# pairlab/SlotFormer

Measured on AMD Instinct MI355X. Metric: rollout frames/sec at B=32, 128x128, 7 slots, 6+50 steps (SAVi-encode + SlotFormer rollout), higher is better.
Workload: dtype f32 storage; matmul/conv on split-bf16 MFMA (bf16x3: hi*hi+hi*lo+lo*hi, f32 accumulate)

## Files before the change

### slotformer_amd/csrc/layer_tok.hip

```cpp
#include "../../include/slotformer_hip.h"
#include "sf_internal.h"
#include "layer_fused.h"
#include "layer_tok_common.h"
#include <stdlib.h>

namespace {
constexpr int LT_NT = 256, LT_D = 256, LT_F = 1024, LT_NH = 8, LT_TOK = 128, LT_MAXL = 8;
constexpr int LT_STAGE = 32 * 1024, LT_RING = 3;
constexpr int LT_NST_ATT = 4 * LT_NH, LT_NST = LT_NST_ATT + 2 * (LT_F / 32);
constexpr int LT_KV = LT_RING * LT_STAGE;
constexpr int LT_VT = LT_KV + 16 * 1024;
constexpr int LT_PAR = LT_KV + 32 * 1024;
constexpr int P_LN1G = 0, P_LN1B = 256, P_BQKV = 512, P_BO = 1280, P_LN2G = 1536, P_LN2B = 1792, P_B1 = 2048, P_B2 = 3072, P_N = 3328;
constexpr size_t LT_LDS = (size_t)LT_PAR + (size_t)P_N * 4;
constexpr size_t LT_BLOB = (size_t)LT_NST * LT_STAGE + (size_t)P_N * 4;
static_assert(LT_LDS <= 160 * 1024, "LDS budget");

struct LtArgs {
  const float* x;
  const float* ring;
  const float* pe;
  float* y;
  const char* blob[LT_MAXL];
  float eps;
  int nl, B, L, vpw, RF, N, f0, dbg_ts;
};
}

__device__ long long lt_ts[16];
#define LTS(i) do { if (A.dbg_ts && blockIdx.x == 0 && threadIdx.x == 0) lt_ts[i] = wall_clock64(); } while (0)

template <int MODE>
__global__ __launch_bounds__(LT_NT) void layer_tok_kernel(LtArgs A) {
  extern __shared__ __attribute__((aligned(16))) char smem[];
  float* P = (float*)(smem + LT_PAR);
  const int t = threadIdx.x, lane = t & 63;
  const int wave = __builtin_amdgcn_readfirstlane(t >> 6);
  const int n = lane & 31, h = lane >> 5;
  const int L = A.L;
  const int v0 = blockIdx.x * A.vpw;
  const int nvalid = min(A.vpw, A.B - v0) * L;
  const int tl = wave * 32 + n;
  const int te = min(tl, nvalid - 1);
  const int vl = te / L, tok = te - vl * L;
  const long long row = (long long)(v0 + vl) * L + tok;
  LTS(0);
  f32x16 X[8];
  if constexpr (MODE == 0) {
    const float* xr = A.x + row * LT_D + 4 * h;
#pragma unroll
    for (int ob = 0; ob < 8; ++ob)
#pragma unroll
      for (int g = 0; g < 4; ++g) {
        const f32x4 v = *(const f32x4*)(xr + 32 * ob + 8 * g);
#pragma unroll
        for (int q = 0; q < 4; ++q) X[ob][4 * g + q] = v[q];
      }
  } else {
    const int fr = tok / A.N, sl = tok - fr * A.N;
    const float* rr = A.ring + (((long long)(v0 + vl) * A.RF + (A.f0 + fr) % A.RF) * A.N + sl) * LT_D + 4 * h;
    const float* pr = A.pe + (long long)tok * LT_D + 4 * h;
#pragma unroll
    for (int ob = 0; ob < 8; ++ob)
#pragma unroll
      for (int g = 0; g < 4; ++g) {
        const f32x4 v = *(const f32x4*)(rr + 32 * ob + 8 * g);
#pragma unroll
        for (int q = 0; q < 4; ++q) X[ob][4 * g + q] = v[q];
      }
    __builtin_amdgcn_sched_barrier(0);
#pragma unroll
    for (int ob = 0; ob < 8; ++ob) {
#pragma unroll
      for (int g = 0; g < 4; ++g) {
        const f32x4 v = *(const f32x4*)(pr + 32 * ob + 8 * g);
#pragma unroll
        for (int q = 0; q < 4; ++q) X[ob][4 * g + q] += v[q];
      }
      __builtin_amdgcn_sched_barrier(0);
    }
  }
  const unsigned wlane = (unsigned)(wave * 8 * 1024 + lane * 16);
  char* const wdst = smem + (wave * 8) * 1024;
  int cur = 0;
  int cs = -2;
  const char* base_cur = A.blob[0];
  const char* base_nxt = A.blob[0];
  bool last_layer = false;
  auto stage_src = [&]() -> const char* {
    const int t2 = cs + 2;
    const bool wrap = t2 >= LT_NST;
    const char* b = wrap ? base_nxt : base_cur;
    const int so = wrap ? (last_layer ? LT_NST - 1 : t2 - LT_NST) : t2;
    ++cs;
    return b + (size_t)so * LT_STAGE + wlane;
  };
  {
    const char* s0 = stage_src();
    const char* s1 = stage_src();
    LtRing R0{nullptr, s0, wdst}, R1{nullptr, s1, wdst + LT_STAGE};
#pragma unroll
    for (int f = 0; f < 8; ++f) lt_dma(R0, f);
#pragma unroll
    for (int f = 0; f < 8; ++f) lt_dma(R1, f);
  }
#ifdef LT_STAMPS
  long long c_wait = 0, c_bar = 0, c_last = 0, c_work = 0;
#endif
  auto stage_begin = [&]() -> LtRing {
#ifdef LT_STAMPS
    const long long c0 = __builtin_readcyclecounter();
    if (c_last) c_work += c0 - c_last;
#endif
#ifdef LT_NODMA
    asm volatile("s_waitcnt vmcnt(0)" ::: "memory");
#else
    asm volatile("s_waitcnt vmcnt(8)" ::: "memory");
#endif
    asm volatile("s_waitcnt lgkmcnt(0)" ::: "memory");
#ifdef LT_STAMPS
    const long long c1 = __builtin_readcyclecounter();
#endif
#ifndef LT_NOBAR
    __builtin_amdgcn_s_barrier();
#endif
    asm volatile("" ::: "memory");
#ifdef LT_STAMPS
    c_last = __builtin_readcyclecounter();
    c_wait += c1 - c0;
    c_bar += c_last - c1;
#endif
    const int nb = cur == 0 ? 2 : cur - 1;
    LtRing R{smem + cur * LT_STAGE + lane * 16, stage_src(), wdst + nb * LT_STAGE};
#ifdef LT_BURST
#pragma unroll
    for (int f = 0; f < 8; ++f) lt_dma_now(R, f);
#endif
    cur = cur == 2 ? 0 : cur + 1;
    return R;
  };
  const int wf = min(wave * 32, nvalid - 1);
  const int kb0 = ((wf / L) * L) >> 5;
  const int d0 = 32 * kb0 + 4 * h - vl * L;
  const char* pb;
  {
    unsigned pbo = (unsigned)(LT_PAR + 16 * h);
    asm volatile("" : "+v"(pbo));
    pb = smem + pbo;
  }
  char* const kwr = smem + LT_KV + wave * 1024 + lane * 16;
  char* const vwr = smem + LT_VT + wave * 4096 + lane * 16;
  const char* krd[3];
  const char* vrd[3];
#pragma unroll
  for (int kbi = 0; kbi < 3; ++kbi) {
    const int kb = min(kb0 + kbi, 3);
    krd[kbi] = smem + LT_KV + kb * 1024 + lane * 16;
    vrd[kbi] = smem + LT_VT + kb * 4096 + lane * 16;
  }
  const float qscale = 0.2550348616841918f;
  constexpr float NEG = -3.0e38f;
  LTS(1);

#pragma unroll 1
  for (int l = 0; l < A.nl; ++l) {
    cs = 0;
    base_cur = A.blob[l];
    last_layer = l + 1 >= A.nl;
    base_nxt = A.blob[last_layer ? l : l + 1];
    __syncthreads();
    {
      const float* vsrc = (const float*)(A.blob[l] + (size_t)LT_NST * LT_STAGE);
      for (int i = t; i < P_N / 4; i += LT_NT) *(f32x4*)(P + 4 * i) = *(const f32x4*)(vsrc + 4 * i);
    }
    __syncthreads();
    if (l == 0) LTS(2);
    bf16x8 xh[16], xl[16];
    lt_layernorm<P_LN1G, P_LN1B>(X, pb, h, A.eps, xh, xl);
    lt_add_vec<P_BO>(X, pb);
    if (l == 0) LTS(3);
    f32x16 qa, ka, va, S[3], O;
    bf16x8 qh[2], ql[2], ph[3][2], pl[3][2], oh[2], ol[2];
    float mx0 = NEG, mx1 = NEG, mx = 0.f, sm = 0.f, rinv = 0.f;
    auto zero16 = [](f32x16& a) {
#pragma unroll
      for (int r = 0; r < 16; ++r) a[r] = 0.f;
    };
    int hq = 0;
    auto mask_chunk = [&](int c) {
      const int kbi = c >> 1;
#pragma unroll
      for (int rr = 0; rr < 8; ++rr) {
        const int r = 8 * (c & 1) + rr;
        const bool ok = (unsigned)(d0 + 32 * kbi + 8 * (r >> 2) + (r & 3)) < (unsigned)L;
        const float v = ok ? S[kbi][r] : NEG;
        S[kbi][r] = v;
        if (rr & 1) mx1 = fmaxf(mx1, v); else mx0 = fmaxf(mx0, v);
      }
    };
    auto exp_chunk = [&](int c) {
      const int kbi = c >> 1;
      float s0 = 0.f, s1 = 0.f;
#pragma unroll
      for (int rr = 0; rr < 8; ++rr) {
        const int r = 8 * (c & 1) + rr;
#ifdef LT_EXPF
        const float e = __expf((S[kbi][r] - mx) * 0.6931471805599453f);
#else
        const float e = __builtin_amdgcn_exp2f(S[kbi][r] - mx);
#endif
        S[kbi][r] = e;
        if (rr & 1) s1 += e; else s0 += e;
      }
      sm += s0 + s1;
    };
    auto psplit_chunk = [&](int c) { split8(quad(S[c >> 1], 2 * (c & 1)), quad(S[c >> 1], 2 * (c & 1) + 1), ph[c >> 1][c & 1], pl[c >> 1][c & 1]); };
    auto kconv = [&](int s) {
      const float* bk = (const float*)pb + P_BQKV + 256 + 32 * hq;
      bf16x8 fh, fl;
      split8(quad(ka, 2 * s) + *(const f32x4*)(bk + 16 * s), quad(ka, 2 * s + 1) + *(const f32x4*)(bk + 16 * s + 8), fh, fl);
      *(bf16x8*)(kwr + (s * 2) * 4096) = fh;
      *(bf16x8*)(kwr + (s * 2 + 1) * 4096) = fl;
    };
    auto qconv = [&](int s) {
      const float* bq = (const float*)pb + P_BQKV + 32 * hq;
      split8((quad(qa, 2 * s) + *(const f32x4*)(bq + 16 * s)) * qscale, (quad(qa, 2 * s + 1) + *(const f32x4*)(bq + 16 * s + 8)) * qscale, qh[s], ql[s]);
    };
    auto vconv = [&](int s) {
      const float bv = P[P_BQKV + 512 + 32 * hq + n];
      bf16x8 fh, fl;
      split8(quad(va, 2 * s) + bv, quad(va, 2 * s + 1) + bv, fh, fl);
      *(bf16x8*)(vwr + (s * 2) * 1024) = fh;
      *(bf16x8*)(vwr + (s * 2 + 1) * 1024) = fl;
    };
    auto oconv = [&](int s) { split8(quad(O, 2 * s) * rinv, quad(O, 2 * s + 1) * rinv, oh[s], ol[s]); };
    auto scores = [&]() {
      bf16x8 kh[3][2], kl[3][2];
#pragma unroll
      for (int kbi = 0; kbi < 3; ++kbi)
#pragma unroll
        for (int s = 0; s < 2; ++s) {
          kh[kbi][s] = *(const bf16x8*)(krd[kbi] + (s * 2) * 4096);
          kl[kbi][s] = *(const bf16x8*)(krd[kbi] + (s * 2 + 1) * 4096);
        }
#pragma unroll
      for (int kbi = 0; kbi < 3; ++kbi) zero16(S[kbi]);
#pragma unroll
      for (int s = 0; s < 2; ++s) {
#pragma unroll
        for (int kbi = 0; kbi < 3; ++kbi) { S[kbi] = LT_MFMA(kh[kbi][s], ql[s], S[kbi]); LT_PIN(); }
#pragma unroll
        for (int kbi = 0; kbi < 3; ++kbi) { S[kbi] = LT_MFMA(kl[kbi][s], qh[s], S[kbi]); LT_PIN(); }
#pragma unroll
        for (int kbi = 0; kbi < 3; ++kbi) { S[kbi] = LT_MFMA(kh[kbi][s], qh[s], S[kbi]); LT_PIN(); }
      }
      mx0 = mx1 = NEG;
      sm = 0.f;
    };
    auto pv = [&]() {
      f32x16 Op[3];
      bf16x8 vh[3][2], vlo[3][2];
#pragma unroll
      for (int kbi = 0; kbi < 3; ++kbi)
#pragma unroll
        for (int s = 0; s < 2; ++s) {
          vh[kbi][s] = *(const bf16x8*)(vrd[kbi] + (s * 2) * 1024);
          vlo[kbi][s] = *(const bf16x8*)(vrd[kbi] + (s * 2 + 1) * 1024);
        }
#pragma unroll
      for (int kbi = 0; kbi < 3; ++kbi) zero16(Op[kbi]);
#pragma unroll
      for (int s = 0; s < 2; ++s) {
#pragma unroll
        for (int kbi = 0; kbi < 3; ++kbi) { Op[kbi] = LT_MFMA(vh[kbi][s], pl[kbi][s], Op[kbi]); LT_PIN(); }
#pragma unroll
        for (int kbi = 0; kbi < 3; ++kbi) { Op[kbi] = LT_MFMA(vlo[kbi][s], ph[kbi][s], Op[kbi]); LT_PIN(); }
#pragma unroll
        for (int kbi = 0; kbi < 3; ++kbi) { Op[kbi] = LT_MFMA(vh[kbi][s], ph[kbi][s], Op[kbi]); LT_PIN(); }
      }
#pragma unroll
      for (int r = 0; r < 16; ++r) O[r] = (Op[0][r] + Op[1][r]) + Op[2][r];
    };
    auto sideD = [&](int g) {
      if (g < 6) mask_chunk(g);
      if (g == 6) mx = lt_xmax(fmaxf(mx0, mx1), h);
      if (g == 7) exp_chunk(0);
    };
    auto sideA = [&](int g) {
      if (g == 0) { exp_chunk(1); exp_chunk(2); }
      if (g == 1) { exp_chunk(3); exp_chunk(4); }
      if (g == 2) { exp_chunk(5); rinv = 1.0f / lt_xsum(sm, h); psplit_chunk(0); }
      if (g == 3) { psplit_chunk(1); psplit_chunk(2); }
      if (g == 4) { psplit_chunk(3); psplit_chunk(4); }
      if (g == 5) psplit_chunk(5);
    };
    {
      const LtRing R = stage_begin();
      lt_row_product<false, 0>(R, xh, xl, qa, LtNoSide{});
    }
    {
      const LtRing R = stage_begin();
      lt_row_product<false, 0>(R, xh, xl, ka, LtNoSide{});
    }
    {
      const LtRing R = stage_begin();
      lt_row_product<true, 5>(R, xh, xl, va, [&](int g) {
        if (g < 2) kconv(g);
        else if (g < 4) qconv(g - 2);
      });
      vconv(0);
      vconv(1);
    }
#pragma unroll 1
    for (hq = 1; hq < LT_NH; ++hq) {
      {
        const LtRing R = stage_begin();
        scores();
          lt_row_product<false, 6>(R, xh, xl, qa, sideD);
      }
      {
        const LtRing R = stage_begin();
          lt_row_product<false, 6>(R, xh, xl, ka, sideA);
        pv();
      }
      {
        const LtRing R = stage_begin();
          lt_row_product<true, 5>(R, xh, xl, va, [&](int g) {
          if (g < 2) kconv(g);
          else if (g < 4) qconv(g - 2);
          else if (g < 6) oconv(g - 4);
        });
      }
      {
        const LtRing R = stage_begin();
        lt_kslice_product<5>(R, oh, ol, X, [&](int g) {
          if (g < 2) vconv(g);
        });
      }
    }
    asm volatile("s_waitcnt lgkmcnt(0)" ::: "memory");
    __builtin_amdgcn_s_barrier();
    asm volatile("" ::: "memory");
    scores();
#pragma unroll
    for (int g = 0; g < 8; ++g) sideD(g);
#pragma unroll
    for (int g = 0; g < 6; ++g) sideA(g);
    pv();
    oconv(0);
    oconv(1);
    {
      const LtRing R = stage_begin();
      lt_kslice_product<0>(R, oh, ol, X, LtNoSide{});
    }
    if (l == 0) LTS(4);
#ifdef LT_STAMPS
    if (l == 0 && blockIdx.x == 0 && threadIdx.x == 0) { lt_ts[8] = c_wait; lt_ts[9] = c_bar; lt_ts[10] = c_work; }
#endif
    lt_layernorm<P_LN2G, P_LN2B>(X, pb, h, A.eps, xh, xl);
    lt_add_vec<P_B2>(X, pb);
    if (l == 0) LTS(5);
    f32x16 Ha, Hb;
    bf16x8 hh[2], hl[2];
    f32x4 b1q[4];
    auto b1_load = [&](int blk) {
      const float* b1 = (const float*)pb + P_B1 + 32 * blk;
#pragma unroll
      for (int g = 0; g < 4; ++g) b1q[g] = *(const f32x4*)(b1 + 8 * g);
    };
    auto hconv = [&](const f32x16& Hx, int s) {
      const f32x4 z4 = {0.f, 0.f, 0.f, 0.f};
      const f32x4 u0 = __builtin_elementwise_max(quad(Hx, 2 * s) + b1q[2 * s], z4);
      const f32x4 u1 = __builtin_elementwise_max(quad(Hx, 2 * s + 1) + b1q[2 * s + 1], z4);
      split8(u0, u1, hh[s], hl[s]);
    };
    auto ffn_step = [&](f32x16& Hn, const f32x16& Hp, int j) {
      {
        const LtRing R = stage_begin();
        lt_row_product<false, 4>(R, xh, xl, Hn, [&](int g) {
          if (g >= 1 && g < 3) hconv(Hp, g - 1);
        });
        asm volatile("" : "+v"(hh[0]), "+v"(hh[1]), "+v"(hl[0]), "+v"(hl[1]));
      }
      {
        const LtRing R = stage_begin();
        b1_load(j);
        lt_kslice_product<0>(R, hh, hl, X, LtNoSide{});
      }
    };
    {
      const LtRing R = stage_begin();
      b1_load(0);
      lt_row_product<false, 0>(R, xh, xl, Ha, LtNoSide{});
    }
    ffn_step(Hb, Ha, 1);
#pragma unroll 1
    for (int j = 2; j < LT_F / 32; j += 2) {
      ffn_step(Ha, Hb, j);
      ffn_step(Hb, Ha, j + 1);
    }
    hconv(Hb, 0);
    hconv(Hb, 1);
    {
      const LtRing R = stage_begin();
      lt_kslice_product<0>(R, hh, hl, X, LtNoSide{});
    }
    if (l == 0) LTS(6);
#ifdef LT_STAMPS
    if (l == 0 && blockIdx.x == 0 && threadIdx.x == 0) { lt_ts[11] = c_wait; lt_ts[12] = c_bar; lt_ts[13] = c_work; }
#endif
  }
  asm volatile("s_waitcnt vmcnt(0)" ::: "memory");
  if (tl < nvalid) {
    float* yr = A.y + row * LT_D + 4 * h;
#pragma unroll
    for (int ob = 0; ob < 8; ++ob)
#pragma unroll
      for (int g = 0; g < 4; ++g) *(f32x4*)(yr + 32 * ob + 8 * g) = quad(X[ob], g);
  }
  LTS(7);
}

extern "C" int sf_debug_read_ts_layer_tok(long long* out16) {
  hipError_t e = hipMemcpyFromSymbol(out16, HIP_SYMBOL(lt_ts), sizeof(long long) * 16);
  return e == hipSuccess ? 0 : (int)e;
}

extern "C" size_t sf_layer_tok_packed_bytes(void) { return LT_BLOB; }
extern "C" size_t sf_layer_tok_packed_bytes_ex(int d_model, int num_heads, int ffn) {
  if (d_model == LT_D && num_heads == LT_NH && ffn == LT_F) return LT_BLOB;
  return sf_layer_tok128_shape(d_model, num_heads, ffn) ? sf_layer_tok128_packed_bytes() : 0;
}

extern "C" int sf_pack_layer_tok_weights(const sf_tfm_layer* w, void* packed, int d_model, int num_heads, int ffn, void* stream) {
  SF_REQUIRE(w && packed, "sf_pack_layer_tok_weights: null pointer");
  SF_REQUIRE(w->in_proj_w && w->out_proj_w && w->lin1_w && w->lin2_w && w->norm1_g && w->norm1_b && w->in_proj_b && w->out_proj_b && w->norm2_g &&
                 w->norm2_b && w->lin1_b && w->lin2_b, "sf_pack_layer_tok_weights: null weight");
  hipStream_t st = (hipStream_t)stream;
  if (sf_layer_tok128_shape(d_model, num_heads, ffn)) return sf_pack_layer_tok128(w, packed, st);
  SF_REQUIRE(d_model == LT_D && num_heads == LT_NH && ffn == LT_F, "sf_pack_layer_tok_weights: (d_model, heads, ffn) = (256, 8, 1024) or (128, 8, 512) only");
  const int total = LT_NST * 32 * 64;
  hipLaunchKernelGGL((pack_layer_tok_kernel<LT_D, LT_F>), dim3((total + 255) / 256), dim3(256), 0, st, w->in_proj_w, w->out_proj_w, w->lin1_w, w->lin2_w, (uint4*)packed);
  SF_CHECK_LAUNCH();
  float* vec = (float*)((char*)packed + (size_t)LT_NST * LT_STAGE);
  const struct {
    const float* src;
    int off, n;
  } parts[8] = {{w->norm1_g, P_LN1G, 256}, {w->norm1_b, P_LN1B, 256}, {w->in_proj_b, P_BQKV, 768}, {w->out_proj_b, P_BO, 256},
                {w->norm2_g, P_LN2G, 256}, {w->norm2_b, P_LN2B, 256}, {w->lin1_b, P_B1, 1024},   {w->lin2_b, P_B2, 256}};
  for (const auto& p : parts) {
    const hipError_t e = hipMemcpyAsync(vec + p.off, p.src, (size_t)p.n * 4, hipMemcpyDeviceToDevice, st);
    if (e != hipSuccess) return sf_set_err((int)e, hipGetErrorString(e), __FILE__, __LINE__);
  }
  return 0;
}

int sf_layer_tok_vpw(int L) {
  if (L < 1 || L > 96) return 0;
  for (int vpw = LT_TOK / L; vpw >= 1; --vpw) {
    const int nvalid = vpw * L;
    bool ok = true;
    for (int w = 0; w < 4 && ok; ++w) {
      const int wf = w * 32 < nvalid ? w * 32 : nvalid - 1, wl = w * 32 + 31 < nvalid ? w * 32 + 31 : nvalid - 1;
      const int kb0 = ((wf / L) * L) >> 5, kb1 = (((wl / L) * L) + L - 1) >> 5;
      ok = kb1 - kb0 + 1 <= 3;
    }
    if (ok) return vpw;
  }
  return 0;
}
bool sf_layer_tok_ok(int L) { return sf_layer_tok_vpw(L) > 0; }

int sf_layer_tok_ex(int mode, const float* xin, const float* ring, int ring_frames, int nslots, int f0, const float* pe, const sf_tfm_layer* layers, int nl,
                    float eps, float* y, int B, int L, hipStream_t st) {
  bool ok = layers && nl >= 1 && nl <= LT_MAXL && sf_layer_tok_ok(L) && B >= 1 && y && (mode == 0 ? xin != nullptr : (ring && pe && nslots >= 1 && ring_frames >= 1));
  for (int l = 0; ok && l < nl; ++l) ok = layers[l].tok_packed != nullptr;
  if (!ok)
    return sf_set_err(-1, "invalid argument: the token-stationary layers need sf_pack_layer_tok_weights fragments, 1..8 layers and 1 <= L <= 96 rows per video", __FILE__, __LINE__);
  static const int dbg = sf_dbg("lt");
  LtArgs A;
  A.x = xin; A.ring = ring; A.pe = pe; A.y = y;
  for (int l = 0; l < LT_MAXL; ++l) A.blob[l] = (const char*)layers[l < nl ? l : nl - 1].tok_packed;
  A.eps = eps; A.nl = nl; A.B = B; A.L = L; A.vpw = sf_layer_tok_vpw(L); A.RF = ring_frames; A.N = nslots; A.f0 = f0; A.dbg_ts = dbg;
  const int nwg = (B + A.vpw - 1) / A.vpw;
  const double flops = nl * ((double)B * L * (2.0 * LT_D * (3 * LT_D + LT_D + 2 * LT_F)) + (double)B * LT_NH * 4.0 * L * L * 32);
  if (mode == 0) {
    SF_TRY(sf_ensure_dyn_lds((const void*)layer_tok_kernel<0>, LT_LDS));
    sf_prof_begin(SF_K_LAYER_TOK, st, flops);
    hipLaunchKernelGGL(layer_tok_kernel<0>, dim3(nwg), dim3(LT_NT), LT_LDS, st, A);
  } else {
    SF_TRY(sf_ensure_dyn_lds((const void*)layer_tok_kernel<1>, LT_LDS));
    sf_prof_begin(SF_K_LAYER_TOK, st, flops);
    hipLaunchKernelGGL(layer_tok_kernel<1>, dim3(nwg), dim3(LT_NT), LT_LDS, st, A);
  }
  sf_prof_end(SF_K_LAYER_TOK, st);
  SF_CHECK_LAUNCH();
  return 0;
}

extern "C" int sf_layer_tok_block_f32(const sf_tfm_layer* w, int nl, const float* x, float* y, int B, int L, void* stream) {
  SF_REQUIRE(w && x && y && B > 0 && nl >= 1 && nl <= LT_MAXL, "sf_layer_tok_block_f32: null pointer / empty problem / more than 8 layers");
  SF_REQUIRE(sf_get_precision() == 1, "sf_layer_tok_block_f32: split-bf16 mode only");
  return sf_layer_tok_ex(0, x, nullptr, 1, 1, 0, nullptr, w, nl, 1e-5f, y, B, L, (hipStream_t)stream);
}

extern "C" int sf_layer_tok_block_ex_f32(const sf_tfm_layer* w, int nl, int d_model, int num_heads, int ffn, const float* x, float* y, int B, int L,
                                         void* stream) {
  SF_REQUIRE(w && x && y && B > 0 && nl >= 1 && nl <= LT_MAXL, "sf_layer_tok_block_ex_f32: null pointer / empty problem / more than 8 layers");
  SF_REQUIRE(sf_get_precision() == 1, "sf_layer_tok_block_ex_f32: split-bf16 mode only");
  if (sf_layer_tok128_shape(d_model, num_heads, ffn)) return sf_layer_tok128_ex(x, w, nl, 1e-5f, y, B, L, (hipStream_t)stream);
  SF_REQUIRE(d_model == LT_D && num_heads == LT_NH && ffn == LT_F, "sf_layer_tok_block_ex_f32: (d_model, heads, ffn) = (256, 8, 1024) or (128, 8, 512) only");
  return sf_layer_tok_ex(0, x, nullptr, 1, 1, 0, nullptr, w, nl, 1e-5f, y, B, L, (hipStream_t)stream);
}
```

Baseline: 669,800.

## Double-buffer per-layer vector params in LDS and prefetch via async global_load_lds

Replaces the per-layer synchronous copy of the LayerNorm/bias vector block (two __syncthreads plus a global-to-LDS loop) with a double-buffered LDS region. The next layer's block is fetched with global_load_lds during the first FFN stage, and the vmcnt waits are adjusted to account for the extra in-flight loads. This removes two block-wide barriers and an exposed global-load latency per layer. In exchange it uses more LDS and makes the vmcnt accounting more delicate.

```diff
diff --git a/slotformer_amd/csrc/layer_tok.hip b/slotformer_amd/csrc/layer_tok.hip
--- a/slotformer_amd/csrc/layer_tok.hip
+++ b/slotformer_amd/csrc/layer_tok.hip
@@ -3,6 +3,7 @@
 #include "layer_fused.h"
 #include "layer_tok_common.h"
 #include <stdlib.h>
+#include <type_traits>
 
 namespace {
 constexpr int LT_NT = 256, LT_D = 256, LT_F = 1024, LT_NH = 8, LT_TOK = 128, LT_MAXL = 8;
@@ -12,7 +13,9 @@
 constexpr int LT_VT = LT_KV + 16 * 1024;
 constexpr int LT_PAR = LT_KV + 32 * 1024;
 constexpr int P_LN1G = 0, P_LN1B = 256, P_BQKV = 512, P_BO = 1280, P_LN2G = 1536, P_LN2B = 1792, P_B1 = 2048, P_B2 = 3072, P_N = 3328;
-constexpr size_t LT_LDS = (size_t)LT_PAR + (size_t)P_N * 4;
+constexpr int LT_PARB = P_N * 4;
+static_assert(LT_PARB % 1024 == 0 && LT_PARB / 1024 == 13, "the vector block is copied as whole 1 KB pieces, three per wave + the last one");
+constexpr size_t LT_LDS = (size_t)LT_PAR + 2 * (size_t)LT_PARB;
 constexpr size_t LT_BLOB = (size_t)LT_NST * LT_STAGE + (size_t)P_N * 4;
 static_assert(LT_LDS <= 160 * 1024, "LDS budget");
 
@@ -33,7 +36,7 @@
 template <int MODE>
 __global__ __launch_bounds__(LT_NT) void layer_tok_kernel(LtArgs A) {
   extern __shared__ __attribute__((aligned(16))) char smem[];
-  float* P = (float*)(smem + LT_PAR);
+  const float* P = (const float*)(smem + LT_PAR);
   const int t = threadIdx.x, lane = t & 63;
   const int wave = __builtin_amdgcn_readfirstlane(t >> 6);
   const int n = lane & 31, h = lane >> 5;
@@ -45,6 +48,19 @@
   const int vl = te / L, tok = te - vl * L;
   const long long row = (long long)(v0 + vl) * L + tok;
   LTS(0);
+  auto vec_dma = [&](const char* blob, int par) {
+    const char* vs = blob + (size_t)LT_NST * LT_STAGE + lane * 16;
+    char* vd = smem + LT_PAR + par * LT_PARB;
+    const void __attribute__((address_space(1)))* s3 = (const void __attribute__((address_space(1)))*)(vs + wave * 3072);
+    void __attribute__((address_space(3)))* d3 = (void __attribute__((address_space(3)))*)(vd + wave * 3072);
+    __builtin_amdgcn_global_load_lds(s3, d3, 16, 0, 0);
+    __builtin_amdgcn_global_load_lds(s3, d3, 16, 1024, 0);
+    __builtin_amdgcn_global_load_lds(s3, d3, 16, 2048, 0);
+    __builtin_amdgcn_global_load_lds((const void __attribute__((address_space(1)))*)(vs + 12 * 1024),
+                                     (void __attribute__((address_space(3)))*)(vd + 12 * 1024), 16, 0, 0);
+    __builtin_amdgcn_sched_barrier(0);
+  };
+  vec_dma(A.blob[0], 0);
   f32x16 X[8];
   if constexpr (MODE == 0) {
     const float* xr = A.x + row * LT_D + 4 * h;
@@ -107,7 +123,7 @@
 #ifdef LT_STAMPS
   long long c_wait = 0, c_bar = 0, c_last = 0, c_work = 0;
 #endif
-  auto stage_begin = [&]() -> LtRing {
+  auto stage_begin_n = [&](auto keep) -> LtRing {
 #ifdef LT_STAMPS
     const long long c0 = __builtin_readcyclecounter();
     if (c_last) c_work += c0 - c_last;
@@ -115,7 +131,8 @@
 #ifdef LT_NODMA
     asm volatile("s_waitcnt vmcnt(0)" ::: "memory");
 #else
-    asm volatile("s_waitcnt vmcnt(8)" ::: "memory");
+    if constexpr (decltype(keep)::value == 12) asm volatile("s_waitcnt vmcnt(12)" ::: "memory");
+    else asm volatile("s_waitcnt vmcnt(8)" ::: "memory");
 #endif
     asm volatile("s_waitcnt lgkmcnt(0)" ::: "memory");
 #ifdef LT_STAMPS
@@ -139,15 +156,11 @@
     cur = cur == 2 ? 0 : cur + 1;
     return R;
   };
+  auto stage_begin = [&]() -> LtRing { return stage_begin_n(std::integral_constant<int, 8>{}); };
   const int wf = min(wave * 32, nvalid - 1);
   const int kb0 = ((wf / L) * L) >> 5;
   const int d0 = 32 * kb0 + 4 * h - vl * L;
   const char* pb;
-  {
-    unsigned pbo = (unsigned)(LT_PAR + 16 * h);
-    asm volatile("" : "+v"(pbo));
-    pb = smem + pbo;
-  }
   char* const kwr = smem + LT_KV + wave * 1024 + lane * 16;
   char* const vwr = smem + LT_VT + wave * 4096 + lane * 16;
   const char* krd[3];
@@ -160,6 +173,13 @@
   }
   const float qscale = 0.2550348616841918f;
   constexpr float NEG = -3.0e38f;
+#if defined(LT_NODMA) || defined(LT_BURST)
+  asm volatile("s_waitcnt vmcnt(0)" ::: "memory");
+#else
+  asm volatile("s_waitcnt vmcnt(16)" ::: "memory");
+#endif
+  __builtin_amdgcn_s_barrier();
+  asm volatile("" ::: "memory");
   LTS(1);
 
 #pragma unroll 1
@@ -168,12 +188,13 @@
     base_cur = A.blob[l];
     last_layer = l + 1 >= A.nl;
     base_nxt = A.blob[last_layer ? l : l + 1];
-    __syncthreads();
-    {
-      const float* vsrc = (const float*)(A.blob[l] + (size_t)LT_NST * LT_STAGE);
-      for (int i = t; i < P_N / 4; i += LT_NT) *(f32x4*)(P + 4 * i) = *(const f32x4*)(vsrc + 4 * i);
-    }
-    __syncthreads();
+    const int par = l & 1;
+    P = (const float*)(smem + LT_PAR + par * LT_PARB);
+    {
+      unsigned pbo = (unsigned)(LT_PAR + par * LT_PARB + 16 * h);
+      asm volatile("" : "+v"(pbo));
+      pb = smem + pbo;
+    }
     if (l == 0) LTS(2);
     bf16x8 xh[16], xl[16];
     lt_layernorm<P_LN1G, P_LN1B>(X, pb, h, A.eps, xh, xl);
@@ -374,9 +395,9 @@
       const f32x4 u1 = __builtin_elementwise_max(quad(Hx, 2 * s + 1) + b1q[2 * s + 1], z4);
       split8(u0, u1, hh[s], hl[s]);
     };
-    auto ffn_step = [&](f32x16& Hn, const f32x16& Hp, int j) {
+    auto ffn_step = [&](f32x16& Hn, const f32x16& Hp, int j, auto keep) {
       {
-        const LtRing R = stage_begin();
+        const LtRing R = stage_begin_n(keep);
         lt_row_product<false, 4>(R, xh, xl, Hn, [&](int g) {
           if (g >= 1 && g < 3) hconv(Hp, g - 1);
         });
@@ -390,14 +411,15 @@
     };
     {
       const LtRing R = stage_begin();
+      vec_dma(base_nxt, par ^ 1);
       b1_load(0);
       lt_row_product<false, 0>(R, xh, xl, Ha, LtNoSide{});
     }
-    ffn_step(Hb, Ha, 1);
+    ffn_step(Hb, Ha, 1, std::integral_constant<int, 12>{});
 #pragma unroll 1
     for (int j = 2; j < LT_F / 32; j += 2) {
-      ffn_step(Ha, Hb, j);
-      ffn_step(Hb, Ha, j + 1);
+      ffn_step(Ha, Hb, j, std::integral_constant<int, 8>{});
+      ffn_step(Hb, Ha, j + 1, std::integral_constant<int, 8>{});
     }
     hconv(Hb, 0);
     hconv(Hb, 1);
```

After: 667,200. About the same (-0.4%).
